# radiocosmology/draco

Hardware: AMD Instinct MI355X
Metric: m-modes/sec through MModeTransform+DirtyMapMaker (128-feed, 256-freq) (higher is better)
Workload: dtype f64 accumulate; B stored complex128; FFT complex64 (as the reference); 1 GPU; cfg3: 128-feed (379 stacked baselines), 256 freq per GPU (256 in the job), 1024 RA, lmax=mmax=512: MModeTransform.process + DirtyMapMaker.process through the task classes (131328 (m,f) solves + alm2map to nside=256 IQUV maps per GPU and day); parallelism=freq-sharded x1, weak scaling (no collective in the timed region)

## Files before the change

### draco_amd/csrc/dense_kernels.h

```cpp
#pragma once
#include <math.h>
#include <string.h>

#include <algorithm>
#include <map>
#include <vector>

#include "dmm_internal.h"

namespace {

typedef double v4d __attribute__((ext_vector_type(4)));

constexpr int kThreads = 256;
constexpr int TB = 64;
constexpr int KC = 16;
constexpr int CPT = KC / 4;
constexpr int LP = 2 * KC + 1;

enum { MODE_GRAM = 0, MODE_UPDATE = 1, MODE_PANEL = 2, MODE_GRAMX = 3 };

struct DenseParams {
  const dmm_tile* tiles;
  int64_t tile0;
  int nmat;
  int N, Np, T;
  const void* B;
  int b_c128, full_layout;
  int gram_dma;
  int npairs, npol, lmax, nfreq;
  const double2* mvis;
  const double* mweight;
  const double* Sl;
  const double* Sk;
  int sk_pitch;
  int add_identity;
  double2* A;
  double2* Linv;
  double2* wbuf;
  int J;
  int sky;
  const double2* X;
  int ldx;
  double2* alm;
  int n_m;
  int* fail;
  const int* msel;
  double* theta;
  double* diag;
  double2* gcache;
  const int* gslot;
  const int32_t* gvalid;
  int64_t xstride;
  int lr_n;
  const int* lr_rank;
};
__device__ __forceinline__ const double2* x_of(const DenseParams& p, int mat) {
  return p.X + (p.xstride ? (int64_t)mat * p.xstride : (int64_t)mat * p.Np * p.ldx);
}

__device__ __forceinline__ void ml_diag_write(const DenseParams& p, const dmm_tile& tile, double cnt, double mnk, double mxc, double smax) {
  __shared__ double s_diag[3][4];
#pragma unroll
  for (int o = 32; o > 0; o >>= 1) {
    cnt += __shfl_xor(cnt, o);
    mnk = fmin(mnk, __shfl_xor(mnk, o));
    mxc = fmax(mxc, __shfl_xor(mxc, o));
  }
  if ((threadIdx.x & 63) == 0) {
    s_diag[0][threadIdx.x >> 6] = cnt;
    s_diag[1][threadIdx.x >> 6] = mnk;
    s_diag[2][threadIdx.x >> 6] = mxc;
  }
  __syncthreads();
  if (threadIdx.x == 0) {
    double* d = p.diag + ((int64_t)tile.f * p.n_m + tile.m) * 4;
    d[0] = s_diag[0][0] + s_diag[0][1] + s_diag[0][2] + s_diag[0][3];
    d[1] = smax;
    d[2] = fmin(fmin(s_diag[1][0], s_diag[1][1]), fmin(s_diag[1][2], s_diag[1][3]));
    d[3] = fmax(fmax(s_diag[2][0], s_diag[2][1]), fmax(s_diag[2][2], s_diag[2][3]));
  }
  __syncthreads();
}

__device__ __forceinline__ double2 load_bc(const void* B, int c128, int64_t off) {
  if (c128) return reinterpret_cast<const double2*>(B)[off];
  const float2 v = reinterpret_cast<const float2*>(B)[off];
  return make_double2((double)v.x, (double)v.y);
}

__device__ __forceinline__ int order_of(const DenseParams& p, const dmm_tile& t) {
  return p.sky ? p.npol * (p.lmax + 1 - t.m) : p.N;
}

__device__ __forceinline__ void fetch_beam_general(double2 (&v)[CPT], const DenseParams& p, const dmm_tile& tile, int row0,
                                                   int k0, int K, bool scale_s) {
  const int r = threadIdx.x >> 2, c0 = (threadIdx.x & 3) * CPT;
  const int row = row0 + r;
  const int L = p.lmax + 1 - tile.m;
  int k = k0 + c0;
  const int pol_stride = p.full_layout ? p.lmax + 1 : L;
  const int64_t rbase = tile.b_off + (int64_t)row * p.npol * pol_stride + (p.full_layout ? tile.m : 0);
  int pol = 0;
  for (int q = 1; q < p.npol; ++q) pol += (k >= q * L);
  int lrel = k - pol * L;
#pragma unroll
  for (int c = 0; c < CPT; ++c, ++k) {
    v[c] = make_double2(0.0, 0.0);
    if (row < p.N && k < K) {
      v[c] = load_bc(p.B, p.b_c128, rbase + (int64_t)pol * pol_stride + lrel);
      if (scale_s && p.Sl) {
        const double sc = p.Sl[tile.m + lrel];
        v[c].x *= sc;
        v[c].y *= sc;
      }
    }
    if (++lrel == L) {
      lrel = 0;
      ++pol;
    }
  }
}

__device__ __forceinline__ void commit(double* lds, const double2 (&v)[CPT]) {
  const int r = threadIdx.x >> 2, c0 = (threadIdx.x & 3) * CPT;
#pragma unroll
  for (int c = 0; c < CPT; ++c) {
    lds[r * LP + 2 * (c0 + c)] = v[c].x;
    lds[r * LP + 2 * (c0 + c) + 1] = v[c].y;
  }
}

template <int MODE>
__global__ __launch_bounds__(kThreads) void k_nt(DenseParams p) {
  __shared__ __align__(16) double xs[TB * LP];
  __shared__ __align__(16) double ys[TB * LP];
  const int mat = blockIdx.y;
  int gs = -1;
  if (MODE == MODE_GRAM && p.gcache) {
    gs = p.gslot[mat];
    if (gs >= 0 && p.gvalid[gs]) return;
  }
  const dmm_tile tile = p.tiles[p.tile0 + mat];
  int bi, bj;
  if (MODE == MODE_GRAM || MODE == MODE_GRAMX) {
    const int tt = blockIdx.x;
    bi = (int)((sqrt(8.0 * tt + 1.0) - 1.0) * 0.5);
    while ((bi + 1) * (bi + 2) / 2 <= tt) ++bi;
    while (bi * (bi + 1) / 2 > tt) --bi;
    bj = tt - bi * (bi + 1) / 2;
  } else if (MODE == MODE_UPDATE) {
    bi = p.J + blockIdx.x;
    bj = p.J;
  } else {
    bi = p.J + 1 + blockIdx.x;
    bj = p.J;
  }
  const int I0 = bi * TB, J0 = bj * TB;
  const int K = MODE == MODE_GRAM    ? p.npol * (p.lmax + 1 - tile.m)
                : MODE == MODE_GRAMX ? 2 * p.npairs
                : MODE == MODE_UPDATE ? p.J * TB
                                      : TB;

  const int lane = threadIdx.x & 63, wave = threadIdx.x >> 6;
  const int quad = (wave + blockIdx.x + blockIdx.y) & 3;
  int wr = quad >> 1, wc = quad & 1;
  const int lr = lane & 15, lk = lane >> 4;
  unsigned tmask = 0xF;
  if (MODE != MODE_PANEL && bi == bj) {
    if (quad == 0 || quad == 3) tmask = 0xD;
    else if (quad == 2) tmask = 0x3;
    else wr = 1, wc = 0, tmask = 0xC;
  }
  const bool dead = false;
  const unsigned emask = tmask;
  const v4d vz = (v4d){0.0, 0.0, 0.0, 0.0};
  v4d c0r = vz, c0i = vz, c1r = vz, c1i = vz, c2r = vz, c2i = vz, c3r = vz, c3i = vz;

  double2 xr[CPT], yr[CPT];
  auto mfma_chunk = [&]() __attribute__((always_inline)) {
    if (dead) return;
    const int sgn = (lk & 1) ? 0 : (int)0x80000000u;
#pragma unroll
    for (int kk = 0; kk < 2 * KC; kk += 4) {
      double a[2], b[2], b2[2];
#pragma unroll
      for (int t = 0; t < 2; ++t) {
        a[t] = xs[(32 * wr + 16 * t + lr) * LP + kk + lk];
        b[t] = ys[(32 * wc + 16 * t + lr) * LP + kk + lk];
        const double o = ys[(32 * wc + 16 * t + lr) * LP + kk + (lk ^ 1)];
        b2[t] = __hiloint2double(__double2hiint(o) ^ sgn, __double2loint(o));
      }
      if (tmask & 1u) {
        c0r = __builtin_amdgcn_mfma_f64_16x16x4f64(a[0], b[0], c0r, 0, 0, 0);
        c0i = __builtin_amdgcn_mfma_f64_16x16x4f64(a[0], b2[0], c0i, 0, 0, 0);
      }
      if (tmask & 2u) {
        c1r = __builtin_amdgcn_mfma_f64_16x16x4f64(a[0], b[1], c1r, 0, 0, 0);
        c1i = __builtin_amdgcn_mfma_f64_16x16x4f64(a[0], b2[1], c1i, 0, 0, 0);
      }
      if (tmask & 4u) {
        c2r = __builtin_amdgcn_mfma_f64_16x16x4f64(a[1], b[0], c2r, 0, 0, 0);
        c2i = __builtin_amdgcn_mfma_f64_16x16x4f64(a[1], b2[0], c2i, 0, 0, 0);
      }
      if (tmask & 8u) {
        c3r = __builtin_amdgcn_mfma_f64_16x16x4f64(a[1], b[1], c3r, 0, 0, 0);
        c3i = __builtin_amdgcn_mfma_f64_16x16x4f64(a[1], b2[1], c3i, 0, 0, 0);
      }
    }
  };
  auto pipeline = [&](auto&& fetch, auto&& finish) {
    if (K > 0) fetch(0);
    for (int k0 = 0; k0 < K; k0 += KC) {
      __syncthreads();
      finish();
      commit(xs, xr);
      commit(ys, yr);
      __syncthreads();
      if (k0 + KC < K) fetch(k0 + KC);
      if (MODE == MODE_PANEL) {
        const int c = k0 / KC;
        tmask = (c <= 2 * wc ? 0x5u : 0u) | (c <= 2 * wc + 1 ? 0xAu : 0u);
      }
      mfma_chunk();
    }
  };

  const int r = threadIdx.x >> 2, c0 = (threadIdx.x & 3) * CPT;
  if (MODE == MODE_GRAM && (p.full_layout || (K & 3) != 0)) {
    pipeline(
        [&](int k0) {
          fetch_beam_general(xr, p, tile, I0, k0, K, false);
          fetch_beam_general(yr, p, tile, J0, k0, K, true);
        },
        [&]() {});
  } else if (MODE == MODE_GRAM && !p.b_c128) {
    const int rx = min(I0 + r, p.N - 1), ry = min(J0 + r, p.N - 1);
    const float2* base = reinterpret_cast<const float2*>(p.B) + tile.b_off;
    const float2* xp = base + (int64_t)rx * K + c0;
    const float2* yp = base + (int64_t)ry * K + c0;
    const double* sk = p.Sk ? p.Sk + (int64_t)tile.m * p.sk_pitch + c0 : nullptr;
    float4 xraw[2], yraw[2];
    double2 sraw[2];
    bool in = true;
    pipeline(
        [&](int k0) {
          in = k0 + c0 < K;
          const int ka = in ? k0 : 0;
          xraw[0] = *reinterpret_cast<const float4*>(xp + ka);
          xraw[1] = *reinterpret_cast<const float4*>(xp + ka + 2);
          yraw[0] = *reinterpret_cast<const float4*>(yp + ka);
          yraw[1] = *reinterpret_cast<const float4*>(yp + ka + 2);
          if (sk) {
            sraw[0] = *reinterpret_cast<const double2*>(sk + k0);
            sraw[1] = *reinterpret_cast<const double2*>(sk + k0 + 2);
          }
        },
        [&]() {
          const double s0 = sk ? sraw[0].x : 1.0, s1 = sk ? sraw[0].y : 1.0, s2 = sk ? sraw[1].x : 1.0, s3 = sk ? sraw[1].y : 1.0;
          const double z = in ? 1.0 : 0.0;
          xr[0] = make_double2(z * (double)xraw[0].x, z * (double)xraw[0].y);
          xr[1] = make_double2(z * (double)xraw[0].z, z * (double)xraw[0].w);
          xr[2] = make_double2(z * (double)xraw[1].x, z * (double)xraw[1].y);
          xr[3] = make_double2(z * (double)xraw[1].z, z * (double)xraw[1].w);
          yr[0] = make_double2(s0 * (double)yraw[0].x, s0 * (double)yraw[0].y);
          yr[1] = make_double2(s1 * (double)yraw[0].z, s1 * (double)yraw[0].w);
          yr[2] = make_double2(s2 * (double)yraw[1].x, s2 * (double)yraw[1].y);
          yr[3] = make_double2(s3 * (double)yraw[1].z, s3 * (double)yraw[1].w);
        });
  } else {
    const double2 *xp, *yp;
    const double* sk = nullptr;
    if (MODE == MODE_GRAM) {
      const double2* base = reinterpret_cast<const double2*>(p.B) + tile.b_off;
      xp = base + (int64_t)min(I0 + r, p.N - 1) * K + c0;
      yp = base + (int64_t)min(J0 + r, p.N - 1) * K + c0;
      if (p.Sk) sk = p.Sk + (int64_t)tile.m * p.sk_pitch + c0;
    } else if (MODE == MODE_GRAMX) {
      const int n = order_of(p, tile);
      xp = x_of(p, mat) + (int64_t)min(I0 + r, n - 1) * p.ldx + c0;
      yp = x_of(p, mat) + (int64_t)min(J0 + r, n - 1) * p.ldx + c0;
    } else if (MODE == MODE_UPDATE) {
      xp = p.A + ((int64_t)mat * p.Np + I0 + r) * p.Np + c0;
      yp = p.A + ((int64_t)mat * p.Np + J0 + r) * p.Np + c0;
    } else {
      xp = p.A + ((int64_t)mat * p.Np + I0 + r) * p.Np + J0 + c0;
      yp = p.Linv + (((int64_t)mat * p.T + p.J) * TB + r) * TB + c0;
    }
    double2 sraw[2];
    pipeline(
        [&](int k0) {
          if (MODE == MODE_UPDATE || MODE == MODE_PANEL || k0 + KC <= K) {
#pragma unroll
            for (int c = 0; c < CPT; ++c) {
              xr[c] = xp[k0 + c];
              yr[c] = yp[k0 + c];
            }
          } else {
#pragma unroll
            for (int c = 0; c < CPT; ++c) {
              const bool in = k0 + c0 + c < K;
              xr[c] = in ? xp[k0 + c] : make_double2(0.0, 0.0);
              yr[c] = in ? yp[k0 + c] : make_double2(0.0, 0.0);
            }
          }
          if (MODE == MODE_GRAM && sk) {
            sraw[0] = *reinterpret_cast<const double2*>(sk + k0);
            sraw[1] = *reinterpret_cast<const double2*>(sk + k0 + 2);
          }
        },
        [&]() {
          if (MODE == MODE_GRAM && sk) {
            yr[0].x *= sraw[0].x, yr[0].y *= sraw[0].x, yr[1].x *= sraw[0].y, yr[1].y *= sraw[0].y;
            yr[2].x *= sraw[1].x, yr[2].y *= sraw[1].x, yr[3].x *= sraw[1].y, yr[3].y *= sraw[1].y;
          }
        });
  }
  if (dead) return;

  const v4d cre[2][2] = {{c0r, c1r}, {c2r, c3r}}, cim[2][2] = {{c0i, c1i}, {c2i, c3i}};
  const int nx = MODE == MODE_GRAMX ? order_of(p, tile) : 0;
#pragma unroll
  for (int ti = 0; ti < 2; ++ti)
#pragma unroll
    for (int tj = 0; tj < 2; ++tj)
#pragma unroll
      for (int reg = 0; reg < 4; ++reg) {
        if (!(emask & (1u << (2 * ti + tj)))) continue;
        const int i = I0 + 32 * wr + 16 * ti + lk + 4 * reg;
        const int j = J0 + 32 * wc + 16 * tj + lr;
        double2* dst = p.A + ((int64_t)mat * p.Np + i) * p.Np + j;
        double re = cre[ti][tj][reg], im = cim[ti][tj][reg];
        if (MODE == MODE_GRAM) {
          if (gs >= 0) p.gcache[((int64_t)gs * gridDim.x + blockIdx.x) * (TB * TB) + (i - I0) * TB + (j - J0)] = make_double2(re, im);
          double di = 0.0, dj = 0.0;
          if (i < p.N) {
            const int s = i >= p.npairs, pp = i - s * p.npairs;
            di = sqrt(p.mweight[(((int64_t)tile.m * 2 + s) * p.nfreq + tile.f) * p.npairs + pp]);
          }
          if (j < p.N) {
            const int s = j >= p.npairs, pp = j - s * p.npairs;
            dj = sqrt(p.mweight[(((int64_t)tile.m * 2 + s) * p.nfreq + tile.f) * p.npairs + pp]);
          }
          re *= di * dj;
          im *= di * dj;
          if (i >= p.N || j >= p.N) re = im = 0.0;
          if (i == j) {
            im = 0.0;
            if (p.add_identity) re += 1.0;
          }
          *dst = make_double2(re, im);
        } else if (MODE == MODE_GRAMX) {
          if (i >= nx || j >= nx) re = im = 0.0;
          if (i == j) im = 0.0;
          *dst = make_double2(re, im);
        } else if (MODE == MODE_UPDATE) {
          const double2 old = *dst;
          *dst = make_double2(old.x - re, old.y - im);
        } else {
          *dst = make_double2(re, im);
        }
      }
}

constexpr int GK = 8;
__device__ __forceinline__ void glds16(const void* g, void* l) {
  __builtin_amdgcn_global_load_lds((const __attribute__((address_space(1))) void*)g, (__attribute__((address_space(3))) void*)l, 16, 0, 0);
}
__global__ __launch_bounds__(kThreads) __attribute__((amdgpu_waves_per_eu(4))) void k_gram_dma(DenseParams p) {
  __shared__ __align__(16) double2 xs[2][TB * GK];
  __shared__ __align__(16) double2 ys[2][TB * GK];
  const int mat = blockIdx.y;
  const dmm_tile tile = p.tiles[p.tile0 + mat];
  const int tt = blockIdx.x;
  int bi = (int)((sqrt(8.0 * tt + 1.0) - 1.0) * 0.5);
  while ((bi + 1) * (bi + 2) / 2 <= tt) ++bi;
  while (bi * (bi + 1) / 2 > tt) --bi;
  const int bj = tt - bi * (bi + 1) / 2;
  const int I0 = bi * TB, J0 = bj * TB;
  const int K = p.npol * (p.lmax + 1 - tile.m);
  const int lane = threadIdx.x & 63, wave = threadIdx.x >> 6;
  const int quad = (wave + blockIdx.x + blockIdx.y) & 3;
  const int wr = quad >> 1, wc = quad & 1;
  const int lr = lane & 15, lk = lane >> 4;
  const bool dead = bi == bj && wc > wr;
  v4d cre[2][2], cim[2][2];
#pragma unroll
  for (int a = 0; a < 2; ++a)
#pragma unroll
    for (int b = 0; b < 2; ++b) cre[a][b] = cim[a][b] = (v4d){0.0, 0.0, 0.0, 0.0};
  const double2* base = reinterpret_cast<const double2*>(p.B) + tile.b_off;
  int xrow[2], yrow[2], kc[2];
#pragma unroll
  for (int j = 0; j < 2; ++j) {
    const int rl = 16 * wave + 8 * j + (lane >> 3);
    kc[j] = (lane & 7) ^ ((rl >> 1) & 7);
    xrow[j] = min(I0 + rl, p.N - 1) * K;
    yrow[j] = min(J0 + rl, p.N - 1) * K;
  }
  const double* sk = p.Sk ? p.Sk + (int64_t)tile.m * p.sk_pitch : nullptr;
  double s[2], sn[2];
  auto issue = [&](int k0, int buf) {
#pragma unroll
    for (int j = 0; j < 2; ++j) {
      const int k = min(k0 + kc[j], K - 1);
      glds16(base + xrow[j] + k, &xs[buf][64 * (2 * wave + j)]);
      glds16(base + yrow[j] + k, &ys[buf][64 * (2 * wave + j)]);
    }
#pragma unroll
    for (int j = 0; j < 2; ++j) {
      const int k = k0 + 4 * j + lk;
      sn[j] = sk ? sk[k] : (k < K ? 1.0 : 0.0);
    }
  };
  issue(0, 0);
  const int sw = (lr >> 1) & 7;
  for (int k0 = 0, buf = 0; k0 < K; k0 += GK, buf ^= 1) {
    __syncthreads();
    s[0] = sn[0], s[1] = sn[1];
    if (k0 + GK < K) issue(k0 + GK, buf ^ 1);
    if (dead) continue;
#pragma unroll
    for (int j = 0; j < 2; ++j) {
      double2 a[2], b[2];
      double nbi[2];
#pragma unroll
      for (int t = 0; t < 2; ++t) {
        a[t] = xs[buf][(32 * wr + 16 * t + lr) * GK + ((4 * j + lk) ^ sw)];
        b[t] = ys[buf][(32 * wc + 16 * t + lr) * GK + ((4 * j + lk) ^ sw)];
        a[t].x *= s[j], a[t].y *= s[j];
        nbi[t] = -b[t].y;
      }
      __builtin_amdgcn_s_setprio(1);
#pragma unroll
      for (int ti = 0; ti < 2; ++ti)
#pragma unroll
        for (int tj = 0; tj < 2; ++tj) {
          cre[ti][tj] = __builtin_amdgcn_mfma_f64_16x16x4f64(a[ti].x, b[tj].x, cre[ti][tj], 0, 0, 0);
          cim[ti][tj] = __builtin_amdgcn_mfma_f64_16x16x4f64(a[ti].y, b[tj].x, cim[ti][tj], 0, 0, 0);
        }
#pragma unroll
      for (int ti = 0; ti < 2; ++ti)
#pragma unroll
        for (int tj = 0; tj < 2; ++tj) {
          cre[ti][tj] = __builtin_amdgcn_mfma_f64_16x16x4f64(a[ti].y, b[tj].y, cre[ti][tj], 0, 0, 0);
          cim[ti][tj] = __builtin_amdgcn_mfma_f64_16x16x4f64(a[ti].x, nbi[tj], cim[ti][tj], 0, 0, 0);
        }
      __builtin_amdgcn_s_setprio(0);
    }
  }
  if (dead) return;
#pragma unroll
  for (int ti = 0; ti < 2; ++ti)
#pragma unroll
    for (int tj = 0; tj < 2; ++tj)
#pragma unroll
      for (int reg = 0; reg < 4; ++reg) {
        const int i = I0 + 32 * wr + 16 * ti + lk + 4 * reg;
        const int j = J0 + 32 * wc + 16 * tj + lr;
        double re = cre[ti][tj][reg], im = cim[ti][tj][reg];
        double di = 0.0, dj = 0.0;
        if (i < p.N) {
          const int sg = i >= p.npairs, pp = i - sg * p.npairs;
          di = sqrt(p.mweight[(((int64_t)tile.m * 2 + sg) * p.nfreq + tile.f) * p.npairs + pp]);
        }
        if (j < p.N) {
          const int sg = j >= p.npairs, pp = j - sg * p.npairs;
          dj = sqrt(p.mweight[(((int64_t)tile.m * 2 + sg) * p.nfreq + tile.f) * p.npairs + pp]);
        }
        re *= di * dj;
        im *= di * dj;
        if (i >= p.N || j >= p.N) re = im = 0.0;
        if (i == j) {
          im = 0.0;
          if (p.add_identity) re += 1.0;
        }
        p.A[((int64_t)mat * p.Np + i) * p.Np + j] = make_double2(re, im);
      }
}
__global__ __launch_bounds__(kThreads) void k_gram_scale(DenseParams p) {
  const int mat = blockIdx.y;
  const int gs = p.gslot[mat];
  if (gs < 0 || !p.gvalid[gs]) return;
  const dmm_tile tile = p.tiles[p.tile0 + mat];
  const int tt = blockIdx.x;
  int bi = (int)((sqrt(8.0 * tt + 1.0) - 1.0) * 0.5);
  while ((bi + 1) * (bi + 2) / 2 <= tt) ++bi;
  while (bi * (bi + 1) / 2 > tt) --bi;
  const int bj = tt - bi * (bi + 1) / 2;
  const int I0 = bi * TB, J0 = bj * TB;
  const double2* src = p.gcache + ((int64_t)gs * gridDim.x + tt) * (TB * TB);
  for (int e = threadIdx.x; e < TB * TB; e += kThreads) {
    const int li = e >> 6, lj = e & 63;
    if (bi == bj && (lj >> 4) > (li >> 4)) continue;
    const int i = I0 + li, j = J0 + lj;
    const double2 raw = src[e];
    double re = raw.x, im = raw.y;
    double di = 0.0, dj = 0.0;
    if (i < p.N) {
      const int s = i >= p.npairs, pp = i - s * p.npairs;
      di = sqrt(p.mweight[(((int64_t)tile.m * 2 + s) * p.nfreq + tile.f) * p.npairs + pp]);
    }
    if (j < p.N) {
      const int s = j >= p.npairs, pp = j - s * p.npairs;
      dj = sqrt(p.mweight[(((int64_t)tile.m * 2 + s) * p.nfreq + tile.f) * p.npairs + pp]);
    }
    re *= di * dj;
    im *= di * dj;
    if (i >= p.N || j >= p.N) re = im = 0.0;
    if (i == j) {
      im = 0.0;
      if (p.add_identity) re += 1.0;
    }
    p.A[((int64_t)mat * p.Np + i) * p.Np + j] = make_double2(re, im);
  }
}
__global__ void k_gram_mark(const int* gslot, int32_t* gvalid, int nmat) {
  const int mat = blockIdx.x * blockDim.x + threadIdx.x;
  if (mat < nmat && gslot[mat] >= 0) gvalid[gslot[mat]] = 1;
}

inline void launch_gram(const DenseParams& p, int nmat, hipStream_t st) {
  const bool dma = p.gram_dma && p.b_c128 && !p.full_layout && (int64_t)p.N * p.npol * (p.lmax + 1) < 0x7fffffff;
  if (dma) hipLaunchKernelGGL(k_gram_dma, dim3(p.T * (p.T + 1) / 2, nmat), dim3(kThreads), 0, st, p);
  else hipLaunchKernelGGL(k_nt<MODE_GRAM>, dim3(p.T * (p.T + 1) / 2, nmat), dim3(kThreads), 0, st, p);
}

__device__ __forceinline__ double fast_rcp(double x) {
  double y = __builtin_amdgcn_rcp(x);
  const double e = __builtin_fma(-x, y, 1.0);
  return __builtin_fma(y, __builtin_fma(e, e, e), y);
}
__device__ __forceinline__ double fast_rsqrt(double x) {
  double y = __builtin_amdgcn_rsq(x);
  const double e = __builtin_fma(-x * y, y, 1.0);
  return __builtin_fma(y * e, __builtin_fma(e, 0.375, 0.5), y);
}

__global__ __launch_bounds__(kThreads) void k_chol_diag(DenseParams p) {
  extern __shared__ __align__(16) unsigned char smem_cd[];
  double2(*a)[TB + 1] = reinterpret_cast<double2(*)[TB + 1]>(smem_cd);
  const int mat = blockIdx.x;
  const int J0 = p.J * TB;
  double2* Ablk = p.A + ((int64_t)mat * p.Np + J0) * p.Np + J0;
  for (int idx = threadIdx.x; idx < TB * TB; idx += kThreads) {
    const int i = idx >> 6, j = idx & 63;
    a[i][j] = j <= i ? Ablk[(int64_t)i * p.Np + j] : make_double2(0.0, 0.0);
  }
  __syncthreads();
  const int ri = threadIdx.x >> 2, rc = threadIdx.x & 3;
  bool bad = false;
  for (int k = 0; k < TB; ++k) {
    const double akk = a[k][k].x;
    bad = bad || !(akk > 0.0);
    if (k > 0 && threadIdx.x < TB) {
      const int i = threadIdx.x;
      const double inv = fast_rsqrt(a[k - 1][k - 1].x);
      if (i > k - 1) {
        a[i][k - 1].x *= inv;
        a[i][k - 1].y *= inv;
      }
    }
    const double rinv = fast_rcp(akk);
    if (ri > k) {
      const double2 x = a[ri][k];
      const double2 xs = make_double2(x.x * rinv, x.y * rinv);
      for (int j = k + 1 + rc; j <= ri; j += 4) {
        const double2 y = a[j][k];
        a[ri][j].x -= xs.x * y.x + xs.y * y.y;
        a[ri][j].y -= xs.y * y.x - xs.x * y.y;
      }
    }
    __syncthreads();
    if (k > 0 && threadIdx.x == 0) a[k - 1][k - 1] = make_double2(sqrt(a[k - 1][k - 1].x), 0.0);
  }
  if (threadIdx.x == 0) {
    a[TB - 1][TB - 1] = make_double2(sqrt(a[TB - 1][TB - 1].x), 0.0);
    if (p.fail && bad) p.fail[mat] = 1;
  }
  __syncthreads();
  __shared__ double dinv[TB];
  if (threadIdx.x < TB) dinv[threadIdx.x] = fast_rcp(a[threadIdx.x][threadIdx.x].x);
  __syncthreads();
  {
    const int j = threadIdx.x >> 2, g = threadIdx.x & 3;
    for (int i = j + 1; i < TB; ++i) {
      double sx = 0.0, sy = 0.0;
      for (int q = j + g; q < i; q += 4) {
        const double2 l = a[i][q];
        const double2 x = q == j ? make_double2(dinv[j], 0.0) : a[j][q];
        sx += l.x * x.x - l.y * x.y;
        sy += l.x * x.y + l.y * x.x;
      }
      sx += __shfl_xor(sx, 1);
      sy += __shfl_xor(sy, 1);
      sx += __shfl_xor(sx, 2);
      sy += __shfl_xor(sy, 2);
      const double inv = dinv[i];
      if (g == 0) a[j][i] = make_double2(-sx * inv, -sy * inv);
      __builtin_amdgcn_wave_barrier();
    }
  }
  __syncthreads();
  double2* Lout = p.Linv + ((int64_t)mat * p.T + p.J) * TB * TB;
  for (int idx = threadIdx.x; idx < TB * TB; idx += kThreads) {
    const int i = idx >> 6, j = idx & 63;
    const double2 zero = make_double2(0.0, 0.0);
    Ablk[(int64_t)i * p.Np + j] = j <= i ? a[i][j] : zero;
    Lout[idx] = j < i ? a[j][i] : (j == i ? make_double2(dinv[i], 0.0) : zero);
  }
}

__global__ __launch_bounds__(kThreads) void k_chol_solve(DenseParams p) {
  extern __shared__ __align__(16) unsigned char smem[];
  double2* y = reinterpret_cast<double2*>(smem);
  double2* t = y + p.Np;
  double2* red = t + TB;
  const int mat = blockIdx.x;
  const dmm_tile tile = p.tiles[p.tile0 + mat];
  const double2* A = p.A + (int64_t)mat * p.Np * p.Np;
  const int Lsky = p.lmax + 1 - tile.m, N = order_of(p, tile);
  for (int i = threadIdx.x; i < p.Np; i += kThreads) {
    double2 b = make_double2(0.0, 0.0);
    if (i < N) {
      if (p.sky) {
        const int pol = i / Lsky, lrel = i - pol * Lsky;
        b = p.alm[(((int64_t)tile.f * p.npol + pol) * p.n_m + tile.m) * (p.lmax + 1) + tile.m + lrel];
      } else {
        const int s = i >= p.npairs, pp = i - s * p.npairs;
        const int64_t o = (((int64_t)tile.m * 2 + s) * p.nfreq + tile.f) * p.npairs + pp;
        const double d = sqrt(p.mweight[o]);
        const double2 v = p.mvis[o];
        b = make_double2(d * v.x, d * v.y);
      }
    }
    y[i] = b;
  }
  __syncthreads();
  const int i64 = threadIdx.x & 63, part = threadIdx.x >> 6;
  for (int J = 0; J < p.T; ++J) {
    const int r = J * TB + i64;
    double sx = 0.0, sy = 0.0;
    for (int k = part; k < J * TB; k += 4) {
      const double2 l = A[(int64_t)r * p.Np + k], z = y[k];
      sx += l.x * z.x - l.y * z.y;
      sy += l.x * z.y + l.y * z.x;
    }
    red[part * TB + i64] = make_double2(sx, sy);
    __syncthreads();
    if (part == 0) {
      double2 s = y[r];
      for (int q = 0; q < 4; ++q) {
        s.x -= red[q * TB + i64].x;
        s.y -= red[q * TB + i64].y;
      }
      t[i64] = s;
    }
    __syncthreads();
    if (part == 0) {
      const double2* Li = p.Linv + (((int64_t)mat * p.T + J) * TB + i64) * TB;
      double zx = 0.0, zy = 0.0;
      for (int q = 0; q <= i64; ++q) {
        const double2 l = Li[q], v = t[q];
        zx += l.x * v.x - l.y * v.y;
        zy += l.x * v.y + l.y * v.x;
      }
      y[r] = make_double2(zx, zy);
    }
    __syncthreads();
  }
  for (int J = p.T - 1; J >= 0; --J) {
    const int c = J * TB + i64;
    double sx = 0.0, sy = 0.0;
    for (int k = (J + 1) * TB + part; k < p.Np; k += 4) {
      const double2 l = A[(int64_t)k * p.Np + c], z = y[k];
      sx += l.x * z.x + l.y * z.y;
      sy += l.x * z.y - l.y * z.x;
    }
// ... 305 lines not shown
```

### draco_amd/csrc/solve_dense.hip

```cpp
#include "dense_kernels.h"
#include "dense_layout.h"
#include "herm_tridiag.h"
#include "herm_band.h"
#ifdef DMM_AB
#include "herm_band_fused.h"
#endif

#define DMM_TRY(call) do { const int rc_ = (call); if (rc_) return rc_; } while (0)

namespace {

template <int KK, int NB>
void td_launch_tri(TdParams& tp, int& np_pend, dim3 grid, hipStream_t st) {
  tp.np = np_pend;
  if (np_pend < NB) {
    hipLaunchKernelGGL((k_td_trail_tri<KK, 0>), grid, dim3(kThreads), 0, st, tp);
  } else {
    hipLaunchKernelGGL((k_td_trail_tri<KK, NB>), grid, dim3(kThreads), 0, st, tp);
    np_pend = 0;
  }
}

void td_launch_trail(TdParams& tp, int& np_pend, int nmat, hipStream_t st) {
  const int n = tp.d.Np, j = tp.j;
// ... 414 lines not shown
  const int mat = blockIdx.y, i = blockIdx.x * blockDim.x + threadIdx.x;
  if (i >= p.Np) return;
  const dmm_tile tile = p.tiles[p.tile0 + mat];
  const int L = p.lmax + 1 - tile.m, N = p.npol * L;
  double2* d = p.A + ((int64_t)mat * p.Np + i) * p.Np + i;
  if (i < N) d->x += 1.0 / Sl[tile.m + i % L];
  else *d = make_double2(1.0, 0.0);
}

namespace dl = dense_layout;
using dl::Layout;
static_assert(dl::kTB == TB && dl::kKC == KC && dl::kC128 == sizeof(double2) && dl::kTileRec == sizeof(dmm_tile), "dense_layout.h and dense_kernels.h disagree");

int64_t workspace_bytes(const dmm_plan* pl, int aux_slots) {
  if (!pl) return 0;
  const Layout L = dl::layout_of(pl->npairs, pl->npol, pl->lmax, aux_slots);
  const int64_t opt = aux_slots >= 2 ? pl->ctx->opt_ml_ws_mib : pl->ctx->opt_wiener_ws_mib;
  return dl::workspace_bytes(L, dl::batch_cap(L, aux_slots, pl->ntile, opt));
}

struct DenseWs {
  Layout L;
  int cap;
  DenseParams base;
  double2* aux;
  double2* blocks;
  double *scale, *theta;
  dmm_tile* tiles;
  int32_t* work;
  int *flag, *slots, *fail, *msel, *any_rot;
};
DenseWs carve_ws(const dmm_plan* pl, int aux_slots, const void* B, const void* mvis, const double* mweight, void* workspace) {
  DenseWs w;
  w.L = dl::layout_of(pl->npairs, pl->npol, pl->lmax, aux_slots);
  w.cap = dl::batch_cap(w.L, aux_slots, pl->ntile, aux_slots >= 2 ? pl->ctx->opt_ml_ws_mib : pl->ctx->opt_wiener_ws_mib);
  const dl::Carve c = dl::carve(w.L, w.cap, aux_slots);
  unsigned char* ws = (unsigned char*)workspace;
  w.aux = (double2*)(ws + c.aux);
  w.blocks = (double2*)(ws + c.blocks);
  w.flag = (int*)(ws + c.flag);
  w.scale = (double*)(ws + c.scale);
  w.theta = (double*)(ws + c.theta);
  w.tiles = (dmm_tile*)(ws + c.tiles);
  w.work = (int32_t*)(ws + c.work);
  w.slots = (int*)(ws + c.slots);
  w.fail = (int*)(ws + c.fail);
  w.msel = (int*)(ws + c.msel);
  w.any_rot = (int*)(ws + c.any_rot);
  DenseParams& p = w.base = DenseParams{};
  p.tiles = pl->tiles_d;
  p.N = w.L.N;
  p.Np = w.L.Np;
  p.T = w.L.T;
  p.B = B;
  p.b_c128 = pl->b_dtype == DMM_C128;
  p.full_layout = pl->b_layout == DMM_B_FULL;
  p.gram_dma = pl->ctx->opt_gram_stage == 1;
  p.npairs = pl->npairs;
  p.npol = pl->npol;
  p.lmax = pl->lmax;
  p.nfreq = pl->nfreq;
  p.mvis = (const double2*)mvis;
  p.mweight = mweight;
  p.A = (double2*)(ws + c.A);
  p.Linv = w.aux;
  p.wbuf = (double2*)(ws + c.wbuf);
  p.n_m = pl->n_m;
  p.diag = pl->ctx->ml_diag;
  return w;
}

struct StreamRestore {
  dmm_ctx* c;
  hipStream_t s;
  ~StreamRestore() { c->stream = s; }
};

void partition_tiles(const dmm_plan* pl, const std::vector<char>& is_null, std::vector<int64_t>& tel_list, std::map<int, std::vector<int64_t>>& sky_lists) {
  const int ntel = 2 * pl->npairs;
  for (int64_t t = 0; t < pl->ntile; ++t) {
    if (!is_null.empty() && is_null[t]) continue;
    const int nsky = pl->npol * (pl->lmax + 1 - pl->tiles_h[t].m);
    if (nsky >= ntel || pl->ctx->opt_ml_shortcut == 3) tel_list.push_back(t);
    else sky_lists[(nsky + TB - 1) / TB * TB].push_back(t);
  }
}

std::vector<int64_t> concat(const std::map<int, std::vector<int64_t>>& lists) {
  std::vector<int64_t> all;
  for (auto& kv : lists) all.insert(all.end(), kv.second.begin(), kv.second.end());
  return all;
}

std::vector<int32_t> gslot_table(const dmm_plan* pl) {
  std::vector<int32_t> gslot_of((size_t)pl->ntile, -1);
  int32_t s = 0;
  for (int64_t t = 0; t < pl->ntile; ++t)
    if (pl->npol * (pl->lmax + 1 - pl->tiles_h[t].m) >= 2 * pl->npairs) gslot_of[(size_t)t] = s++;
  return gslot_of;
}

DenseParams batch_params(const DenseWs& W, size_t off, int nmat, bool sky, int np_sky, void* alm) {
  DenseParams p = W.base;
  p.A = W.base.A + off * W.L.Np * W.L.Np;
  p.wbuf = W.base.wbuf + off * W.L.N;
  p.tiles = W.tiles + off;
  p.tile0 = 0;
  p.nmat = nmat;
  p.sky = sky ? 1 : 0;
  p.N = sky ? np_sky : W.L.N;
  p.Np = (p.N + TB - 1) / TB * TB;
  p.T = p.Np / TB;
  p.alm = (double2*)alm;
  return p;
}

int upload_lists(dmm_plan* pl, const int64_t* ids, int nmat, std::vector<dmm_tile>& tiles_c, std::vector<int32_t>& work_c, dmm_tile* tiles_d,
                 int32_t* work_d, hipStream_t S) {
  dmm_dirty_tile_list(pl, ids, nmat, tiles_c, work_c);
  DMM_HIP(hipMemcpyAsync(tiles_d, tiles_c.data(), nmat * sizeof(dmm_tile), hipMemcpyHostToDevice, S));
  DMM_HIP(hipMemcpyAsync(work_d, work_c.data(), (nmat + 1) * sizeof(int32_t), hipMemcpyHostToDevice, S));
  return DMM_OK;
}
int upload_slots(const std::vector<int32_t>& gslot_of, const int64_t* ids, int nmat, std::vector<int>& slots_c, int* slots_d, hipStream_t S) {
  slots_c.resize(nmat);
  for (int i = 0; i < nmat; ++i) slots_c[i] = gslot_of[(size_t)ids[i]];
  DMM_HIP(hipMemcpyAsync(slots_d, slots_c.data(), nmat * sizeof(int), hipMemcpyHostToDevice, S));
  return DMM_OK;
}

void form_gram(dmm_ctx* ctx, DenseParams& p, int nmat, hipStream_t S, double2* X, const std::vector<int>* slots, const int* slots_d,
               const dmm_tile* count_tiles) {
  const int ntel = 2 * p.npairs, T = p.T;
  auto flops = [&](const dmm_tile& t) {
    const double nsky = (double)p.npol * (p.lmax + 1 - t.m);
    const double k = std::min<double>(ntel, nsky), K = std::max<double>(ntel, nsky);
    return (int64_t)(4.0 * k * k * K);
  };
  for (int i = 0; count_tiles && i < nmat; ++i) ctx->ml_gram_flops += flops(count_tiles[i]);
  if (p.sky) {
    p.ldx = ntel;
    p.X = X;
    hipLaunchKernelGGL(k_xpose, dim3((p.N + 31) / 32, (ntel + 31) / 32, nmat), dim3(kThreads), 0, S, p, X);
    hipLaunchKernelGGL(k_nt<MODE_GRAMX>, dim3(T * (T + 1) / 2, nmat), dim3(kThreads), 0, S, p);
  } else if (slots) {
    for (int i = 0; i < nmat; ++i)
      if ((*slots)[i] >= 0 && ctx->ml_gvalid_h[(size_t)(*slots)[i]]) {
        ++ctx->ml_gram_cached;
        if (count_tiles) ctx->ml_gram_flops -= flops(count_tiles[i]);
      }
    p.gcache = ctx->ml_gcache;
    p.gslot = slots_d;
    p.gvalid = ctx->ml_gvalid;
    hipLaunchKernelGGL(k_nt<MODE_GRAM>, dim3(T * (T + 1) / 2, nmat), dim3(kThreads), 0, S, p);
    hipLaunchKernelGGL(k_gram_scale, dim3(T * (T + 1) / 2, nmat), dim3(kThreads), 0, S, p);
    hipLaunchKernelGGL(k_gram_mark, dim3((nmat + 255) / 256), dim3(256), 0, S, slots_d, ctx->ml_gvalid, nmat);
    for (int i = 0; i < nmat; ++i)
      if ((*slots)[i] >= 0) ctx->ml_gvalid_h[(size_t)(*slots)[i]] = 1;
    p.gcache = nullptr;
  } else {
    launch_gram(p, nmat, S);
  }
}

constexpr size_t kDiagLds = (size_t)TB * (TB + 1) * sizeof(double2);
size_t solve_lds(const Layout& L) { return ((size_t)L.Np + TB + 4 * TB) * sizeof(double2); }
void chol_factor(dmm_ctx* ctx, DenseParams& p, int nmat, hipStream_t S, size_t solve_lds = 0) {
  dmm_prof_scope prof(ctx, DMM_PROF_CHOL, S);
  const int T = p.T;
  for (int J = 0; J < T; ++J) {
    p.J = J;
    if (J > 0) hipLaunchKernelGGL(k_nt<MODE_UPDATE>, dim3(T - J, nmat), dim3(kThreads), 0, S, p);
    hipLaunchKernelGGL(k_chol_diag, dim3(nmat), dim3(kThreads), kDiagLds, S, p);
    if (J < T - 1) hipLaunchKernelGGL(k_nt<MODE_PANEL>, dim3(T - J - 1, nmat), dim3(kThreads), 0, S, p);
  }
  if (solve_lds) hipLaunchKernelGGL(k_chol_solve, dim3(nmat), dim3(kThreads), solve_lds, S, p);
}
int chol_attributes(const Layout& L) {
  DMM_HIP(hipFuncSetAttribute((const void*)k_chol_solve, hipFuncAttributeMaxDynamicSharedMemorySize, (int)solve_lds(L)));
  DMM_HIP(hipFuncSetAttribute((const void*)k_chol_diag, hipFuncAttributeMaxDynamicSharedMemorySize, (int)kDiagLds));
  return DMM_OK;
}

int sky_rhs(dmm_plan* pl, const void* B, const void* mvis, const double* mweight, void* alm,
            const std::map<int, std::vector<int64_t>>& sky_lists, const DenseWs& W) {
  const std::vector<int64_t> all = concat(sky_lists);
  std::vector<dmm_tile> tiles_c;
  std::vector<int32_t> work_c;
  hipStream_t st = pl->ctx->stream;
  for (size_t i0 = 0; i0 < all.size(); i0 += W.cap) {
    const int nmat = (int)std::min<size_t>(W.cap, all.size() - i0);
    DMM_TRY(upload_lists(pl, all.data() + i0, nmat, tiles_c, work_c, W.tiles, W.work, st));
    DMM_HIP(hipStreamSynchronize(st));
    DMM_TRY(dmm_dirty_launch_list(pl, B, mvis, mweight, W.tiles, W.work, nmat, work_c[nmat], alm));
    DMM_HIP(hipStreamSynchronize(st));
  }
  return DMM_OK;
}

TdParams td_params(const dmm_ctx* ctx, const DenseParams& p, const Layout& L, double2* vec, double2* log, int* fail, double acond, double rcond,
                   const int* msel, int tri, int two_stage, double stop_tol) {
  const int n = p.Np;
  TdParams tp;
  tp.d = p;
  tp.d.msel = msel;
  tp.vec = vec;
  tp.log_cs = log;
  tp.log_stride = (int64_t)2 * L.Np * L.Np;
  const int runs = 16 * n;
  tp.run_cap = ctx->opt_ml_eigen == 3 ? -runs : runs;
  tp.log_cap = (int)std::min<int64_t>(tp.log_stride - ((int64_t)3 * runs * sizeof(int) + 15) / 16, 0x7fffffff);
  tp.acond = acond;
  tp.rcond = rcond;
  tp.fail = fail;
  tp.tri = tri;
  tp.two_stage = two_stage;
  tp.nb = sb_pending(ctx, n, tp.log_stride);
  tp.one_block = ctx->opt_ml_reduce == 3 ? 1 : 0;
  tp.fused = ctx->opt_ml_reduce == 5 ? 1 : 0;
  tp.stop_tol = stop_tol;
  tp.bs_U = nullptr;
  if (tp.two_stage) tp.log_cap = (int)std::min<int64_t>(sb_log_cap(tp.log_stride, n, runs), 0x7fffffff);
  return tp;
}

void pair_orders(std::map<int, std::vector<int64_t>>& lists) {
  std::map<int, std::vector<int64_t>> out;
  for (auto it = lists.rbegin(); it != lists.rend(); ++it) {
    auto nx = std::next(it);
    if (nx != lists.rend() && it->second.size() < 600 && nx->second.size() < 600 && it->first - nx->first <= TB) {
      std::vector<int64_t>& d = out[it->first];
      d = it->second;
      d.insert(d.end(), nx->second.begin(), nx->second.end());
      it = nx;
    } else {
      out[it->first] = it->second;
    }
  }
  lists.swap(out);
}

constexpr size_t kSubLds = (size_t)2 * TB * (TB + 1) * sizeof(double2);

struct MlPass {
  dmm_plan* pl;
  dmm_ctx* ctx;
  const void* B;
  void* alm;
  double acond, rcond;
  DenseWs W;
  int ntel, cap, capE, E, cap_direct;
  bool bs_build, bs_use, gcache_on, shortcut;
  std::vector<int32_t> gslot_of;
  std::vector<dmm_tile> tiles_c;
  std::vector<int32_t> work_c;
  std::vector<int> fail_h, msel_h, td_fail_h;
  std::vector<int64_t> tel_deferred;
  std::map<int, std::vector<int64_t>> sky_deferred;

  enum SlotLayout { kHalves, kEarlySlots } slot_layout = kHalves;
  int slot_off(int h) const { return slot_layout == kEarlySlots ? cap_direct + h * E : h * capE; }
  int slot_cap(int h) const { return slot_layout == kEarlySlots ? E : capE; }
  struct Half {
    std::vector<dmm_tile> tiles;
    std::vector<int32_t> work;
    std::vector<int64_t> ids;
    std::vector<int> slots;
    int nmat = 0, off = 0, np = 0, np_sky = 0;
    bool sky = false, busy = false;
  } half[2];
  int chunk_no = 0;
  bool early_used[2] = {false, false};
  std::vector<int64_t> redo_tel;
  std::map<int, std::vector<int64_t>> redo_sky;
  int batch_no = 0;

  MlPass(dmm_plan* pl_, const void* B_, const void* mvis, const double* mweight, double acond_, double rcond_, void* workspace, void* alm_)
      : pl(pl_), ctx(pl_->ctx), B(B_), alm(alm_), acond(acond_), rcond(rcond_), W(carve_ws(pl_, 2, B_, mvis, mweight, workspace)) {
    ntel = W.L.N;
    cap = W.cap;
    const bool bs_have = ctx->ml_bs_U != nullptr && ctx->opt_ml_shortcut != 3 && ctx->opt_ml_reduce == 0 && sb_stop_tol(ctx) > 0.0 &&
                         sb_usable(ctx, W.L.Np) && dmm_ml_gram_cache_slots(pl) <= ctx->ml_bs_slots;
    bs_build = bs_have && ctx->ml_bs_build;
    bs_use = bs_have && !ctx->ml_bs_build && (int64_t)ctx->ml_bs_rank_h.size() >= dmm_ml_gram_cache_slots(pl);
    gcache_on = !bs_build && ctx->ml_gcache && ctx->opt_gram_stage != 1 && ctx->opt_ml_shortcut != 3 && dmm_ml_gram_cache_slots(pl) <= ctx->ml_gslots;
    shortcut = ctx->opt_ml_shortcut != 2 && !bs_build;
    capE = cap / 2;
    E = std::min(128, cap / 8);
    cap_direct = E >= 8 ? cap - 2 * E : cap;
  }

  double sweep_bytes(int n, int k) const {
    const int nb = sb_pending(ctx, n, (int64_t)2 * W.L.Np * W.L.Np);
    const double t = (n - ((8 * (k + 1)) & ~15)) / 16;
    return t * (t + 1) / 2 * (k > 0 && k % nb == 0 ? 8.5 : 4.5) * 1024;
  }
  void count_band(int n, int nmat) {
    double by = 0.0;
    for (int k = 0; k < n / 8 - 1; ++k) by += sweep_bytes(n, k);
    ctx->ml_band_bytes += (int64_t)(by * nmat);
  }
  void count_stop(int n, int ne) {
    ++ctx->ml_order_hist[std::min(((ne ? ne : n) + 63) / 64, 16)];
    if (!ne) return;
    double by = 0.0;
    for (int k = ne / 8 - 1; k < n / 8 - 1; ++k) by += sweep_bytes(n, k);
    ctx->ml_band_bytes -= (int64_t)by;
// ... 676 lines not shown
```

Measured before the change: 2090 m-modes/s.

## Use 3-multiply complex product in Gram MFMA kernels and specialize staging

Replaces the 4-real-MFMA complex multiply-accumulate in the k_nt and k_gram_dma Gram kernels with a Gauss/Karatsuba-style 3-MFMA form (p=ar*br, q=ai*bi, s=(ar+ai)(br-bi)), recombining real and imaginary parts at store time. This cuts MFMA work per k-step by a quarter at the cost of four more accumulator vectors and extra adds. It also templatizes k_nt on the staging path (C128/C64/general) so each variant carries only the code it needs, and lowers the waves_per_eu hint to 3 to leave room for the extra registers. The 3-mult form adds some cancellation error in f64, and the general path may launch two kernels, each of which returns early for tiles it does not own.

```diff
diff --git a/draco_amd/csrc/dense_kernels.h b/draco_amd/csrc/dense_kernels.h
--- a/draco_amd/csrc/dense_kernels.h
+++ b/draco_amd/csrc/dense_kernels.h
@@ -19,6 +19,7 @@
 constexpr int LP = 2 * KC + 1;
 
 enum { MODE_GRAM = 0, MODE_UPDATE = 1, MODE_PANEL = 2, MODE_GRAMX = 3 };
+enum { STAGE_C128 = 0, STAGE_C64 = 1, STAGE_GENERAL = 2 };
 
 struct DenseParams {
   const dmm_tile* tiles;
@@ -131,8 +132,8 @@
   }
 }
 
-template <int MODE>
-__global__ __launch_bounds__(kThreads) void k_nt(DenseParams p) {
+template <int MODE, int STAGE = STAGE_C128>
+__global__ __launch_bounds__(kThreads) __attribute__((amdgpu_waves_per_eu(3))) void k_nt(DenseParams p) {
   __shared__ __align__(16) double xs[TB * LP];
   __shared__ __align__(16) double ys[TB * LP];
   const int mat = blockIdx.y;
@@ -161,6 +162,7 @@
                 : MODE == MODE_GRAMX ? 2 * p.npairs
                 : MODE == MODE_UPDATE ? p.J * TB
                                       : TB;
+  if (MODE == MODE_GRAM && (STAGE == STAGE_GENERAL) != (p.full_layout || (K & 3) != 0)) return;
 
   const int lane = threadIdx.x & 63, wave = threadIdx.x >> 6;
   const int quad = (wave + blockIdx.x + blockIdx.y) & 3;
@@ -175,37 +177,42 @@
   const bool dead = false;
   const unsigned emask = tmask;
   const v4d vz = (v4d){0.0, 0.0, 0.0, 0.0};
-  v4d c0r = vz, c0i = vz, c1r = vz, c1i = vz, c2r = vz, c2i = vz, c3r = vz, c3i = vz;
+  v4d c0p = vz, c0q = vz, c0s = vz, c1p = vz, c1q = vz, c1s = vz, c2p = vz, c2q = vz, c2s = vz, c3p = vz, c3q = vz, c3s = vz;
 
   double2 xr[CPT], yr[CPT];
   auto mfma_chunk = [&]() __attribute__((always_inline)) {
     if (dead) return;
-    const int sgn = (lk & 1) ? 0 : (int)0x80000000u;
-#pragma unroll
-    for (int kk = 0; kk < 2 * KC; kk += 4) {
-      double a[2], b[2], b2[2];
+#pragma unroll
+    for (int kk = 0; kk < 2 * KC; kk += 8) {
+      double ar[2], ai[2], as[2], br[2], bi[2], bd[2];
 #pragma unroll
       for (int t = 0; t < 2; ++t) {
-        a[t] = xs[(32 * wr + 16 * t + lr) * LP + kk + lk];
-        b[t] = ys[(32 * wc + 16 * t + lr) * LP + kk + lk];
-        const double o = ys[(32 * wc + 16 * t + lr) * LP + kk + (lk ^ 1)];
-        b2[t] = __hiloint2double(__double2hiint(o) ^ sgn, __double2loint(o));
+        ar[t] = xs[(32 * wr + 16 * t + lr) * LP + kk + 2 * lk];
+        ai[t] = xs[(32 * wr + 16 * t + lr) * LP + kk + 2 * lk + 1];
+        br[t] = ys[(32 * wc + 16 * t + lr) * LP + kk + 2 * lk];
+        bi[t] = ys[(32 * wc + 16 * t + lr) * LP + kk + 2 * lk + 1];
+        as[t] = ar[t] + ai[t];
+        bd[t] = br[t] - bi[t];
       }
       if (tmask & 1u) {
-        c0r = __builtin_amdgcn_mfma_f64_16x16x4f64(a[0], b[0], c0r, 0, 0, 0);
-        c0i = __builtin_amdgcn_mfma_f64_16x16x4f64(a[0], b2[0], c0i, 0, 0, 0);
+        c0p = __builtin_amdgcn_mfma_f64_16x16x4f64(ar[0], br[0], c0p, 0, 0, 0);
+        c0q = __builtin_amdgcn_mfma_f64_16x16x4f64(ai[0], bi[0], c0q, 0, 0, 0);
+        c0s = __builtin_amdgcn_mfma_f64_16x16x4f64(as[0], bd[0], c0s, 0, 0, 0);
       }
       if (tmask & 2u) {
-        c1r = __builtin_amdgcn_mfma_f64_16x16x4f64(a[0], b[1], c1r, 0, 0, 0);
-        c1i = __builtin_amdgcn_mfma_f64_16x16x4f64(a[0], b2[1], c1i, 0, 0, 0);
+        c1p = __builtin_amdgcn_mfma_f64_16x16x4f64(ar[0], br[1], c1p, 0, 0, 0);
+        c1q = __builtin_amdgcn_mfma_f64_16x16x4f64(ai[0], bi[1], c1q, 0, 0, 0);
+        c1s = __builtin_amdgcn_mfma_f64_16x16x4f64(as[0], bd[1], c1s, 0, 0, 0);
       }
       if (tmask & 4u) {
-        c2r = __builtin_amdgcn_mfma_f64_16x16x4f64(a[1], b[0], c2r, 0, 0, 0);
-        c2i = __builtin_amdgcn_mfma_f64_16x16x4f64(a[1], b2[0], c2i, 0, 0, 0);
+        c2p = __builtin_amdgcn_mfma_f64_16x16x4f64(ar[1], br[0], c2p, 0, 0, 0);
+        c2q = __builtin_amdgcn_mfma_f64_16x16x4f64(ai[1], bi[0], c2q, 0, 0, 0);
+        c2s = __builtin_amdgcn_mfma_f64_16x16x4f64(as[1], bd[0], c2s, 0, 0, 0);
       }
       if (tmask & 8u) {
-        c3r = __builtin_amdgcn_mfma_f64_16x16x4f64(a[1], b[1], c3r, 0, 0, 0);
-        c3i = __builtin_amdgcn_mfma_f64_16x16x4f64(a[1], b2[1], c3i, 0, 0, 0);
+        c3p = __builtin_amdgcn_mfma_f64_16x16x4f64(ar[1], br[1], c3p, 0, 0, 0);
+        c3q = __builtin_amdgcn_mfma_f64_16x16x4f64(ai[1], bi[1], c3q, 0, 0, 0);
+        c3s = __builtin_amdgcn_mfma_f64_16x16x4f64(as[1], bd[1], c3s, 0, 0, 0);
       }
     }
   };
@@ -227,14 +234,14 @@
   };
 
   const int r = threadIdx.x >> 2, c0 = (threadIdx.x & 3) * CPT;
-  if (MODE == MODE_GRAM && (p.full_layout || (K & 3) != 0)) {
+  if (MODE == MODE_GRAM && STAGE == STAGE_GENERAL) {
     pipeline(
         [&](int k0) {
           fetch_beam_general(xr, p, tile, I0, k0, K, false);
           fetch_beam_general(yr, p, tile, J0, k0, K, true);
         },
         [&]() {});
-  } else if (MODE == MODE_GRAM && !p.b_c128) {
+  } else if (MODE == MODE_GRAM && STAGE == STAGE_C64) {
     const int rx = min(I0 + r, p.N - 1), ry = min(J0 + r, p.N - 1);
     const float2* base = reinterpret_cast<const float2*>(p.B) + tile.b_off;
     const float2* xp = base + (int64_t)rx * K + c0;
@@ -318,7 +325,7 @@
   }
   if (dead) return;
 
-  const v4d cre[2][2] = {{c0r, c1r}, {c2r, c3r}}, cim[2][2] = {{c0i, c1i}, {c2i, c3i}};
+  const v4d cp[2][2] = {{c0p, c1p}, {c2p, c3p}}, cq[2][2] = {{c0q, c1q}, {c2q, c3q}}, cs[2][2] = {{c0s, c1s}, {c2s, c3s}};
   const int nx = MODE == MODE_GRAMX ? order_of(p, tile) : 0;
 #pragma unroll
   for (int ti = 0; ti < 2; ++ti)
@@ -330,7 +337,8 @@
         const int i = I0 + 32 * wr + 16 * ti + lk + 4 * reg;
         const int j = J0 + 32 * wc + 16 * tj + lr;
         double2* dst = p.A + ((int64_t)mat * p.Np + i) * p.Np + j;
-        double re = cre[ti][tj][reg], im = cim[ti][tj][reg];
+        const double pp_ = cp[ti][tj][reg], qq_ = cq[ti][tj][reg];
+        double re = pp_ + qq_, im = cs[ti][tj][reg] - pp_ + qq_;
         if (MODE == MODE_GRAM) {
           if (gs >= 0) p.gcache[((int64_t)gs * gridDim.x + blockIdx.x) * (TB * TB) + (i - I0) * TB + (j - J0)] = make_double2(re, im);
           double di = 0.0, dj = 0.0;
@@ -367,7 +375,7 @@
 __device__ __forceinline__ void glds16(const void* g, void* l) {
   __builtin_amdgcn_global_load_lds((const __attribute__((address_space(1))) void*)g, (__attribute__((address_space(3))) void*)l, 16, 0, 0);
 }
-__global__ __launch_bounds__(kThreads) __attribute__((amdgpu_waves_per_eu(4))) void k_gram_dma(DenseParams p) {
+__global__ __launch_bounds__(kThreads) __attribute__((amdgpu_waves_per_eu(3))) void k_gram_dma(DenseParams p) {
   __shared__ __align__(16) double2 xs[2][TB * GK];
   __shared__ __align__(16) double2 ys[2][TB * GK];
   const int mat = blockIdx.y;
@@ -384,11 +392,11 @@
   const int wr = quad >> 1, wc = quad & 1;
   const int lr = lane & 15, lk = lane >> 4;
   const bool dead = bi == bj && wc > wr;
-  v4d cre[2][2], cim[2][2];
+  v4d cp[2][2], cq[2][2], cs[2][2];
 #pragma unroll
   for (int a = 0; a < 2; ++a)
 #pragma unroll
-    for (int b = 0; b < 2; ++b) cre[a][b] = cim[a][b] = (v4d){0.0, 0.0, 0.0, 0.0};
+    for (int b = 0; b < 2; ++b) cp[a][b] = cq[a][b] = cs[a][b] = (v4d){0.0, 0.0, 0.0, 0.0};
   const double2* base = reinterpret_cast<const double2*>(p.B) + tile.b_off;
   int xrow[2], yrow[2], kc[2];
 #pragma unroll
@@ -423,28 +431,23 @@
 #pragma unroll
     for (int j = 0; j < 2; ++j) {
       double2 a[2], b[2];
-      double nbi[2];
+      double as[2], bd[2];
 #pragma unroll
       for (int t = 0; t < 2; ++t) {
         a[t] = xs[buf][(32 * wr + 16 * t + lr) * GK + ((4 * j + lk) ^ sw)];
         b[t] = ys[buf][(32 * wc + 16 * t + lr) * GK + ((4 * j + lk) ^ sw)];
         a[t].x *= s[j], a[t].y *= s[j];
-        nbi[t] = -b[t].y;
+        as[t] = a[t].x + a[t].y;
+        bd[t] = b[t].x - b[t].y;
       }
       __builtin_amdgcn_s_setprio(1);
 #pragma unroll
       for (int ti = 0; ti < 2; ++ti)
 #pragma unroll
         for (int tj = 0; tj < 2; ++tj) {
-          cre[ti][tj] = __builtin_amdgcn_mfma_f64_16x16x4f64(a[ti].x, b[tj].x, cre[ti][tj], 0, 0, 0);
-          cim[ti][tj] = __builtin_amdgcn_mfma_f64_16x16x4f64(a[ti].y, b[tj].x, cim[ti][tj], 0, 0, 0);
-        }
-#pragma unroll
-      for (int ti = 0; ti < 2; ++ti)
-#pragma unroll
-        for (int tj = 0; tj < 2; ++tj) {
-          cre[ti][tj] = __builtin_amdgcn_mfma_f64_16x16x4f64(a[ti].y, b[tj].y, cre[ti][tj], 0, 0, 0);
-          cim[ti][tj] = __builtin_amdgcn_mfma_f64_16x16x4f64(a[ti].x, nbi[tj], cim[ti][tj], 0, 0, 0);
+          cp[ti][tj] = __builtin_amdgcn_mfma_f64_16x16x4f64(a[ti].x, b[tj].x, cp[ti][tj], 0, 0, 0);
+          cq[ti][tj] = __builtin_amdgcn_mfma_f64_16x16x4f64(a[ti].y, b[tj].y, cq[ti][tj], 0, 0, 0);
+          cs[ti][tj] = __builtin_amdgcn_mfma_f64_16x16x4f64(as[ti], bd[tj], cs[ti][tj], 0, 0, 0);
         }
       __builtin_amdgcn_s_setprio(0);
     }
@@ -458,7 +461,8 @@
       for (int reg = 0; reg < 4; ++reg) {
         const int i = I0 + 32 * wr + 16 * ti + lk + 4 * reg;
         const int j = J0 + 32 * wc + 16 * tj + lr;
-        double re = cre[ti][tj][reg], im = cim[ti][tj][reg];
+        const double pp_ = cp[ti][tj][reg], qq_ = cq[ti][tj][reg];
+        double re = pp_ + qq_, im = cs[ti][tj][reg] - pp_ + qq_;
         double di = 0.0, dj = 0.0;
         if (i < p.N) {
           const int sg = i >= p.npairs, pp = i - sg * p.npairs;
@@ -520,10 +524,17 @@
   if (mat < nmat && gslot[mat] >= 0) gvalid[gslot[mat]] = 1;
 }
 
+inline void launch_nt_gram(const DenseParams& p, int nmat, hipStream_t st) {
+  const dim3 grid(p.T * (p.T + 1) / 2, nmat);
+  if (p.full_layout || (p.npol & 3) != 0) hipLaunchKernelGGL((k_nt<MODE_GRAM, STAGE_GENERAL>), grid, dim3(kThreads), 0, st, p);
+  if (p.full_layout) return;
+  if (p.b_c128) hipLaunchKernelGGL((k_nt<MODE_GRAM, STAGE_C128>), grid, dim3(kThreads), 0, st, p);
+  else hipLaunchKernelGGL((k_nt<MODE_GRAM, STAGE_C64>), grid, dim3(kThreads), 0, st, p);
+}
 inline void launch_gram(const DenseParams& p, int nmat, hipStream_t st) {
   const bool dma = p.gram_dma && p.b_c128 && !p.full_layout && (int64_t)p.N * p.npol * (p.lmax + 1) < 0x7fffffff;
   if (dma) hipLaunchKernelGGL(k_gram_dma, dim3(p.T * (p.T + 1) / 2, nmat), dim3(kThreads), 0, st, p);
-  else hipLaunchKernelGGL(k_nt<MODE_GRAM>, dim3(p.T * (p.T + 1) / 2, nmat), dim3(kThreads), 0, st, p);
+  else launch_nt_gram(p, nmat, st);
 }
 
 __device__ __forceinline__ double fast_rcp(double x) {
diff --git a/draco_amd/csrc/solve_dense.hip b/draco_amd/csrc/solve_dense.hip
--- a/draco_amd/csrc/solve_dense.hip
+++ b/draco_amd/csrc/solve_dense.hip
@@ -590,7 +590,7 @@
     p.gcache = ctx->ml_gcache;
     p.gslot = slots_d;
     p.gvalid = ctx->ml_gvalid;
-    hipLaunchKernelGGL(k_nt<MODE_GRAM>, dim3(T * (T + 1) / 2, nmat), dim3(kThreads), 0, S, p);
+    launch_nt_gram(p, nmat, S);
     hipLaunchKernelGGL(k_gram_scale, dim3(T * (T + 1) / 2, nmat), dim3(kThreads), 0, S, p);
     hipLaunchKernelGGL(k_gram_mark, dim3((nmat + 255) / 256), dim3(256), 0, S, slots_d, ctx->ml_gvalid, nmat);
     for (int i = 0; i < nmat; ++i)
```

Result: no change. 2089 m-modes/s (-0.0%).
